# mkocabas/EpipolarPose

Hardware: AMD Instinct MI355X
Metric: images/sec (4-view 256x256, ResNet-50) at 1/2/4/8 MI355X; MPJPE vs ref (higher is better)
Workload: dtype bf16; 1 GPU; configs[1]: ResNet-50 Integral-pose, 4-view 256x256 synthetic, batch=32/GPU, fully-supervised SmoothL1 loss; global_batch=32, joints=17, depth_res=64, optimizer=adam, parallelism=dp1, launch=eager, streams=2, deterministic=True

## Files before the change

### epipolarpose_amd/csrc/common.h

```cpp
#pragma once
#include <hip/hip_runtime.h>
#include <stdint.h>
#include <float.h>
#include "../../include/epipolar_hip.h"

#define EPI_WAVE 64
#define EPI_HD __host__ __device__
#define EPI_LOG2E 1.4426950408889634f

#define EPI_CHECK_LAUNCH()                                   \
    do {                                                     \
        if (hipGetLastError() != hipSuccess) return EPI_ERR_LAUNCH; \
    } while (0)

namespace epi {

typedef float float4v __attribute__((ext_vector_type(4)));
typedef unsigned int uint4v __attribute__((ext_vector_type(4)));

bool deterministic();
float* det_scratch(size_t floats, hipStream_t stream);

__device__ __forceinline__ float fast_exp2(float x) { return __builtin_amdgcn_exp2f(x); }

// ... 35 lines not shown
    __device__ static __forceinline__ void store(unsigned short* p, const float (&v)[8]) {
        unsigned int w[4];
#pragma unroll
        for (int i = 0; i < 4; ++i)
            w[i] = pack_bf16x2(v[2 * i], v[2 * i + 1]);
        uint4v t; t.x = w[0]; t.y = w[1]; t.z = w[2]; t.w = w[3];
        *reinterpret_cast<uint4v*>(p) = t;
    }
    __device__ static __forceinline__ float load1(const unsigned short* p) { return bf16_to_f32(*p); }
    __device__ static __forceinline__ void store1(unsigned short* p, float v) { *p = f32_to_bf16(v); }
};

__device__ __forceinline__ float wave_sum(float v) {
#pragma unroll
    for (int o = 32; o > 0; o >>= 1) v += __shfl_xor(v, o, 64);
    return v;
}
__device__ __forceinline__ float wave_max(float v) {
#pragma unroll
    for (int o = 32; o > 0; o >>= 1) v = fmaxf(v, __shfl_xor(v, o, 64));
    return v;
}

__device__ __forceinline__ float block_sum(float v, float* smem ) {
    const int lane = threadIdx.x & 63, wid = threadIdx.x >> 6, nw = (blockDim.x + 63) >> 6;
    v = wave_sum(v);
    __syncthreads();
    if (lane == 0) smem[wid] = v;
    __syncthreads();
    float t = (lane < nw) ? smem[lane] : 0.f;
    t = wave_sum(t);
    return t;
}

}
```

### epipolarpose_amd/csrc/head_gemm.hip

```cpp
#include "common.h"
#include "bn_affine.h"
#include <algorithm>
#include <cstdlib>
#include <mutex>
#include <type_traits>
#include <unordered_map>
#include <utility>
#include <vector>

namespace epi {

typedef __bf16 bf16x8 __attribute__((ext_vector_type(8)));
typedef float f32x16 __attribute__((ext_vector_type(16)));

constexpr int GBK = 64;

template <int TM_, int WM_, int WN_, int MIN_WAVES_, int NSTAGE_, bool STAGGER_ = false> struct GemmCfg {
    static constexpr int TM = TM_, WM = WM_, WN = WN_, NW = WM_ * WN_, THREADS = 64 * NW, MIN_WAVES = MIN_WAVES_, NSTAGE = NSTAGE_;
    static constexpr bool STAGGER = STAGGER_;
    static constexpr int BM = WM_ * TM_ * 32, BN = WN_ * 64;
    static constexpr int A_BYTES = BM * 128, B_BYTES = BN * 128, STAGE_BYTES = A_BYTES + B_BYTES;
    static constexpr int AP = BM / 8 / NW, BP = BN / 8 / NW;
    static constexpr bool EARLY = NW == 4 && NSTAGE_ == 2;
    static_assert(AP >= 1 && BP >= 1 && BM % (8 * NW) == 0 && BN % (8 * NW) == 0, "whole pieces per wave");
// ... 102 lines not shown
        c.sh[4 * h] = sh.x; c.sh[4 * h + 1] = sh.y; c.sh[4 * h + 2] = sh.z; c.sh[4 * h + 3] = sh.w;
    }
}
__device__ __forceinline__ uint4v bnred_apply(const GemmBnRed& br, uint4v o, uint4v zv, uint4v yv, const BnRedCols& c, float (&s)[8], float (&q)[8]);
__device__ __forceinline__ uint4v bnred_row(const GemmBnRed& br, uint4v o, long long off, const BnRedCols& c, float (&s)[8], float (&q)[8]) {
    const uint4v zv = *reinterpret_cast<const uint4v*>(br.z + off);
    uint4v yv = uint4v{0u, 0u, 0u, 0u};
    if (br.relu && br.y) yv = *reinterpret_cast<const uint4v*>(br.y + off);
    return bnred_apply(br, o, zv, yv, c, s, q);
}
__device__ __forceinline__ uint4v bnred_apply(const GemmBnRed& br, uint4v o, uint4v zv, uint4v yv, const BnRedCols& c, float (&s)[8], float (&q)[8]) {
    unsigned int ow[4] = {o.x, o.y, o.z, o.w};
    const unsigned int zw[4] = {zv.x, zv.y, zv.z, zv.w}, yw[4] = {yv.x, yv.y, yv.z, yv.w};
#pragma unroll
    for (int k = 0; k < 4; ++k) {
#pragma unroll
        for (int h = 0; h < 2; ++h) {
            const int e = 2 * k + h;
            const unsigned int keep = h ? 0xffff0000u : 0x0000ffffu;
            const float g = __uint_as_float(h ? (ow[k] & 0xffff0000u) : (ow[k] << 16));
            const float xv = __uint_as_float(h ? (zw[k] & 0xffff0000u) : (zw[k] << 16));
            bool on = true;
            if (br.relu) on = br.y ? (__uint_as_float(h ? (yw[k] & 0xffff0000u) : (yw[k] << 16)) > 0.f) : (xv * c.sc[e] + c.sh[e] > 0.f);
            const float dz = on ? g : 0.f;
            s[e] += dz;
            q[e] = fmaf(dz, (xv - c.mu[e]) * c.rs[e], q[e]);
            if (!on) ow[k] &= ~keep;
        }
    }
    uint4v r; r.x = ow[0]; r.y = ow[1]; r.z = ow[2]; r.w = ow[3];
    return r;
}

#ifdef EPI_GEMM_TRACE
constexpr int GEMM_TRACE_WGS = 8192, GEMM_TRACE_SLOTS = 16;
__device__ unsigned long long epi_gemm_trace[GEMM_TRACE_WGS * GEMM_TRACE_SLOTS];
#define GEMM_STAMP_V(i, v)                                                                                               \
    do {                                                                                                                 \
        const int wg_ = blockIdx.x + gridDim.x * (blockIdx.y + gridDim.y * blockIdx.z);                                  \
        if (threadIdx.x == 0 && wg_ < GEMM_TRACE_WGS) epi_gemm_trace[wg_ * GEMM_TRACE_SLOTS + (i)] = (v);               \
    } while (0)
#define GEMM_STAMP(i) GEMM_STAMP_V(i, __builtin_amdgcn_s_memtime())
#else
#define GEMM_STAMP_V(i, v) do {} while (0)
#define GEMM_STAMP(i) do {} while (0)
#endif
// ... 114 lines not shown
                for (int k = 0; k < 4; ++k) {
                    const float a = __uint_as_float(w4[k] << 16), b = __uint_as_float(w4[k] & 0xffff0000u);
                    ssum[2 * k] += a; ssq[2 * k] = fmaf(a, a, ssq[2 * k]);
                    ssum[2 * k + 1] += b; ssq[2 * k + 1] = fmaf(b, b, ssq[2 * k + 1]);
                }
            }
            uint4v o; o.x = lo.x; o.y = lo.y; o.z = hi.x; o.w = hi.y;
            if (ADD) o = add_bf16x8(o, AD_EARLY ? ad[it] : addend_at(m_first + 8 * it, off));
            if (RED) o = RED_EARLY ? bnred_apply(p.br, o, zpre[it], ypre[it], rcols, ssum, ssq) : bnred_row(p.br, o, off, rcols, ssum, ssq);
            uint4v* dst = reinterpret_cast<uint4v*>(reinterpret_cast<unsigned short*>(p.C) + off);
            if (nt_stores) __builtin_nontemporal_store(o, dst);
            else *dst = o;
        }
    };
    const bool has_stats = !RED && p.stats != nullptr;
    auto copy_sc = [&](auto sc_c) __attribute__((always_inline)) {
        if (has_stats) { if (has_add) copy_rows(std::true_type{}, std::true_type{}, sc_c); else copy_rows(std::true_type{}, std::false_type{}, sc_c); }
        else if (has_add) copy_rows(std::false_type{}, std::true_type{}, sc_c);
        else copy_rows(std::false_type{}, std::false_type{}, sc_c);
    };
    if (scatter) copy_sc(std::true_type{}); else copy_sc(std::false_type{});
    GEMM_STAMP(6);
    if (has_stats || RED) {
#pragma unroll
        for (int k = 0; k < 8; ++k) {
#pragma unroll
            for (int o = 8; o < 64; o <<= 1) { ssum[k] += __shfl_xor(ssum[k], o, 64); ssq[k] += __shfl_xor(ssq[k], o, 64); }
        }
        float* st = reinterpret_cast<float*>(smem + WM * WN * (TM * 32 * 128));
        if (lane < 8) {
            float* row = st + wm * (2 * GBN) + wn * 64 + c8 * 8;
            *reinterpret_cast<float4v*>(row) = float4v{ssum[0], ssum[1], ssum[2], ssum[3]};
            *reinterpret_cast<float4v*>(row + 4) = float4v{ssum[4], ssum[5], ssum[6], ssum[7]};
            *reinterpret_cast<float4v*>(row + GBN) = float4v{ssq[0], ssq[1], ssq[2], ssq[3]};
            *reinterpret_cast<float4v*>(row + GBN + 4) = float4v{ssq[4], ssq[5], ssq[6], ssq[7]};
        }
        __syncthreads();
        float* dst = RED ? p.br.sums : p.stats + (long long)(tile_m % p.stats_copies) * 2 * p.N;
        for (int t = tid; t < 2 * GBN; t += THREADS) {
            float v = 0.f;
#pragma unroll
            for (int w = 0; w < WM; ++w) v += st[w * (2 * GBN) + t];
            const int which = t / GBN, col = n0 + (t % GBN);
            if (col < p.N) atomicAdd(dst + which * p.N + col, v);
        }
    }
#ifdef EPI_GEMM_TRACE
    asm volatile("s_waitcnt vmcnt(0)" ::: "memory");
    GEMM_STAMP(7);
    GEMM_STAMP_V(8, __builtin_amdgcn_s_memrealtime());
#endif
}

enum { A_PLAIN = 0, A_GATHER = 1, A_PHASED = 2 };


__device__ __forceinline__ bf16x8 bn_in_apply(bf16x8 a, const float4v (&t)[4]) {
    const uint4v u = __builtin_bit_cast(uint4v, a);
    const unsigned int w[4] = {u.x, u.y, u.z, u.w};
// ... 375 lines not shown
                        float* c = reinterpret_cast<float*>(p.C) + orow * p.ldc + n;
                        if (n + 3 < p.N) { float4v t; t.x = v[0]; t.y = v[1]; t.z = v[2]; t.w = v[3]; *reinterpret_cast<float4v*>(c) = t; }
                        else for (int e = 0; e < 4 && n + e < p.N; ++e) c[e] = v[e];
                    } else {
                        unsigned short* c = reinterpret_cast<unsigned short*>(p.C) + orow * p.ldc + n;
                        if (p.addend)
                            for (int e = 0; e < 4 && n + e < p.N; ++e) v[e] = bf16_to_f32(f32_to_bf16(v[e])) + bf16_to_f32(p.addend[orow * p.ldc + n + e]);
                        if (n + 3 < p.N) {
                            uint2 t;
                            t.x = pack_bf16x2(v[0], v[1]);
                            t.y = pack_bf16x2(v[2], v[3]);
                            *reinterpret_cast<uint2*>(c) = t;
                        } else for (int e = 0; e < 4 && n + e < p.N; ++e) c[e] = f32_to_bf16(v[e]);
                    }
                }
            }
        }
    }
}

constexpr int AS_WAVES = 8, AS_LOADERS = 2, AS_RING = 3;
constexpr int AS_THREADS = 64 * (AS_WAVES + AS_LOADERS), AS_BM = 32 * AS_WAVES, AS_BN = 64;

template <int KSTEPS>
__global__ __launch_bounds__(AS_THREADS, 1) void head_gemm_astat_kernel(GemmArgs p) {
    constexpr int K = 16 * KSTEPS, ROW_BYTES = 2 * K, CHUNKS = ROW_BYTES / 16;
    constexpr int BTILE = AS_BN * ROW_BYTES;
    constexpr int ROWS_PER_PIECE = 1024 / ROW_BYTES, PIECES = BTILE / 1024 / AS_LOADERS;
    extern __shared__ __attribute__((aligned(16))) char smem[];
    const int tid = threadIdx.x, lane = tid & 63, wid = tid >> 6;
    const bool loader = wid >= AS_WAVES;
    const int frow = lane & 31, fhalf = lane >> 5;
    const int m0 = xcd_remap(blockIdx.x, gridDim.x) * AS_BM + wid * 32;
    const int n_tiles = (p.N + AS_BN - 1) / AS_BN;
    const char* zero_src = reinterpret_cast<const char*>(epi_zero_chunk);
    float* bias_s = reinterpret_cast<float*>(smem + AS_RING * BTILE + AS_WAVES * 4096);
    float* stats_s = bias_s + n_tiles * AS_BN;
    for (int n = tid; n < n_tiles * AS_BN; n += AS_THREADS) bias_s[n] = (p.bias && n < p.N) ? p.bias[n] : 0.f;
    if (p.stats)
        for (int n = tid; n < 2 * n_tiles * AS_BN; n += AS_THREADS) stats_s[n] = 0.f;

    auto issue_b = [&](int nt) {
        const int lw = wid - AS_WAVES;
        char* dst = smem + (nt % AS_RING) * BTILE + lw * (PIECES * 1024);
#pragma unroll 8
        for (int q = 0; q < PIECES; ++q) {
            const int r = (lw * PIECES + q) * ROWS_PER_PIECE + lane / CHUNKS;
            const int chunk = (lane % CHUNKS) ^ (r % CHUNKS);
            const int n = nt * AS_BN + r;
            const void* src = n < p.N ? reinterpret_cast<const void*>(p.Bt + (long long)n * p.ldb + chunk * 8)
                                      : reinterpret_cast<const void*>(zero_src);
            glds16(src, dst + q * 1024);
        }
    };
    bf16x8 af[KSTEPS];
    if (loader) {
        issue_b(0);
        if (n_tiles > 1) issue_b(1);
    } else {
        const int m = m0 + frow;
        const uint4v* arow = reinterpret_cast<const uint4v*>(p.A + (long long)(m < p.M ? m : 0) * p.lda) + fhalf;
#pragma unroll
        for (int ks = 0; ks < KSTEPS; ++ks) {
            uint4v v = arow[2 * ks];
            if (m >= p.M) v.x = v.y = v.z = v.w = 0u;
            af[ks] = __builtin_bit_cast(bf16x8, v);
        }
    }
    __syncthreads();
    if (loader) {
        for (int nt = 0; nt < n_tiles; ++nt) {
            if (nt + 2 < n_tiles) {
                issue_b(nt + 2);
                asm volatile("s_waitcnt vmcnt(%0)\n\ts_barrier" ::"n"(PIECES) : "memory");
            } else {
                asm volatile("s_waitcnt vmcnt(0)\n\ts_barrier" ::: "memory");
            }
        }
        if (p.stats) __builtin_amdgcn_s_barrier();
        return;
    }
    char* stage = smem + AS_RING * BTILE + wid * 4096;
    const int c8 = lane & 7;
    auto slices = [&](auto add_c, auto stats_c) __attribute__((always_inline)) {
    constexpr bool ADD = decltype(add_c)::value, STATS = decltype(stats_c)::value;
    for (int nt = 0; nt < n_tiles; ++nt) {
        f32x16 acc[2];
#pragma unroll
        for (int j = 0; j < 2; ++j)
#pragma unroll
            for (int r = 0; r < 16; ++r) acc[j][r] = 0.f;
        const unsigned slice_off = (unsigned)(nt % AS_RING) * BTILE;
        auto read_b = [&](int ks, uint4v (&f)[2]) {
#pragma unroll
            for (int tj = 0; tj < 2; ++tj) {
                const int r = tj * 32 + frow;
                const unsigned off = (slice_off + r * ROW_BYTES + (((fhalf ^ r) % CHUNKS) << 4)) ^ (unsigned)(((2 * ks) % CHUNKS) << 4);
                f[tj] = *reinterpret_cast<const uint4v*>(smem + off);
            }
        };
        uint4v ad[4];
        auto load_addend = [&]() {
            if (!ADD) return;
#pragma unroll
            for (int it = 0; it < 4; ++it) {
                const int m = m0 + it * 8 + (lane >> 3), nn = nt * AS_BN + (lane & 7) * 8;
                ad[it] = (m < p.M && nn < p.N) ? *reinterpret_cast<const uint4v*>(p.addend + (long long)m * p.ldc + nn) : uint4v{0u, 0u, 0u, 0u};
            }
        };
        if (KSTEPS <= 8) load_addend();
        uint4v fb[3][2];
        read_b(0, fb[0]);
        if (KSTEPS > 1) read_b(1, fb[1]);
#pragma unroll
        for (int ks = 0; ks < KSTEPS; ++ks) {
            if (ks + 2 < KSTEPS) read_b(ks + 2, fb[(ks + 2) % 3]);
            __builtin_amdgcn_sched_barrier(0);
#pragma unroll
            for (int tj = 0; tj < 2; ++tj)
                acc[tj] = __builtin_amdgcn_mfma_f32_32x32x16_bf16(__builtin_bit_cast(bf16x8, fb[ks % 3][tj]), af[ks], acc[tj], 0, 0, 0);
        }
        asm volatile("s_waitcnt lgkmcnt(0)\n\ts_barrier" ::: "memory");
        const int n0 = nt * AS_BN;
#pragma unroll
        for (int tj = 0; tj < 2; ++tj)
#pragma unroll
            for (int q = 0; q < 4; ++q) {
                const int nl = tj * 32 + 8 * q + 4 * fhalf;
                const float4v bv = *reinterpret_cast<const float4v*>(bias_s + n0 + nl);
                const float v0 = acc[tj][4 * q] + bv.x, v1 = acc[tj][4 * q + 1] + bv.y, v2 = acc[tj][4 * q + 2] + bv.z,
                            v3 = acc[tj][4 * q + 3] + bv.w;
                uint2 t;
                t.x = pack_bf16x2(v0, v1);
                t.y = pack_bf16x2(v2, v3);
                const int unit = tj * 8 + 2 * q + fhalf;
                *reinterpret_cast<uint2*>(stage + frow * 128 + ((unit ^ (frow & 15)) << 3)) = t;
            }
        const int n = n0 + c8 * 8;
        float ssum[8], ssq[8];
#pragma unroll
        for (int k = 0; k < 8; ++k) { ssum[k] = 0.f; ssq[k] = 0.f; }
#pragma unroll
        for (int it = 0; it < 4; ++it) {
            const int row = it * 8 + (lane >> 3), sw = row & 15;
            const uint2 lo = *reinterpret_cast<const uint2*>(stage + row * 128 + (((2 * c8) ^ sw) << 3));
            const uint2 hi = *reinterpret_cast<const uint2*>(stage + row * 128 + (((2 * c8 + 1) ^ sw) << 3));
            const int m = m0 + row;
            if (m < p.M && n < p.N) {
                uint4v o; o.x = lo.x; o.y = lo.y; o.z = hi.x; o.w = hi.y;
                if (ADD) o = add_bf16x8(o, KSTEPS <= 8 ? ad[it] : *reinterpret_cast<const uint4v*>(p.addend + (long long)m * p.ldc + n));
                *reinterpret_cast<uint4v*>(reinterpret_cast<unsigned short*>(p.C) + (long long)m * p.ldc + n) = o;
                if (STATS) {
                    const unsigned int w4[4] = {lo.x, lo.y, hi.x, hi.y};
#pragma unroll
                    for (int k = 0; k < 4; ++k) {
                        const float a = __uint_as_float(w4[k] << 16), b = __uint_as_float(w4[k] & 0xffff0000u);
                        ssum[2 * k] += a; ssq[2 * k] = fmaf(a, a, ssq[2 * k]);
                        ssum[2 * k + 1] += b; ssq[2 * k + 1] = fmaf(b, b, ssq[2 * k + 1]);
                    }
                }
            }
        }
        if (STATS) {
#pragma unroll
            for (int k = 0; k < 8; ++k) {
#pragma unroll
                for (int o = 8; o < 64; o <<= 1) { ssum[k] += __shfl_xor(ssum[k], o, 64); ssq[k] += __shfl_xor(ssq[k], o, 64); }
            }
            if (lane < 8) {
#pragma unroll
                for (int k = 0; k < 8; ++k) {
                    atomicAdd(stats_s + n + k, ssum[k]);
                    atomicAdd(stats_s + n_tiles * AS_BN + n + k, ssq[k]);
                }
            }
        }
    }
    };
    if (p.addend) { if (p.stats) slices(std::true_type{}, std::true_type{}); else slices(std::true_type{}, std::false_type{}); }
    else if (p.stats) slices(std::false_type{}, std::true_type{});
    else slices(std::false_type{}, std::false_type{});
    if (p.stats) {
        asm volatile("s_waitcnt lgkmcnt(0)\n\ts_barrier" ::: "memory");
        float* dst = p.stats + (long long)(blockIdx.x % p.stats_copies) * 2 * p.N;
        for (int n = tid; n < p.N; n += 64 * AS_WAVES) {
            atomicAdd(dst + n, stats_s[n]);
            atomicAdd(dst + p.N + n, stats_s[n_tiles * AS_BN + n]);
        }
    }
}

template <int TM_, int WM_, int WN_> struct PatchCfg {
    static constexpr int TM = TM_, WM = WM_, WN = WN_, NW = WM_ * WN_, THREADS = 64 * NW;
    static constexpr int BM = WM_ * TM_ * 32, BN = WN_ * 64, B_BYTES = BN * 128, BP = BN / 8 / NW;
    static_assert(NW == 8 && BP >= 1, "8 waves");
};
typedef PatchCfg<2, 4, 2> PatchWide;
typedef PatchCfg<1, 8, 1> PatchNarrow;
typedef PatchCfg<1, 4, 2> PatchHalf;
constexpr int PATCH_TAPS = 9, PATCH_APW = 8;

#ifdef EPI_PATCH_TRACE
__device__ unsigned long long epi_patch_trace[64 * 96];
#define PATCH_STAMP(i)                                                                                                   \
    do {                                                                                                                 \
        const int wg_ = blockIdx.x + gridDim.x * blockIdx.y;                                                             \
        if (lane == 0 && wid == 0 && wg_ % 16 == 0 && wg_ / 16 < 64 && (i) < 96) epi_patch_trace[(wg_ / 16) * 96 + (i)] = __builtin_amdgcn_s_memtime(); \
// ... 261 lines not shown
static int g_pipe_force_fwd();
static int gemm_pipe_mode() {
    const int v = 0;
    const int f = g_pipe_force_fwd();
    return f >= 0 ? f : v;
}

static int g_store_policy = -1;
static int gemm_store_policy() {
    if (g_store_policy < 0) g_store_policy = 0;
    return g_store_policy;
}
extern "C" int epi_gemm_store_policy(int v) {
    const int before = gemm_store_policy();
    if (v >= 0) g_store_policy = v;
    return before;
}
static int g_tile_force = 0, g_pipe_force = -1;
extern "C" int epi_gemm_tune(int tile, int pipe) {
    if (tile >= 0) g_tile_force = tile;
    if (pipe >= -1) g_pipe_force = pipe;
    return g_tile_force;
}

static int g_tile_force_fwd() { return g_tile_force; }
static int g_pipe_force_fwd() { return g_pipe_force; }

static GemmPlan gemm_plan_cfg(int cfg, int M, int N, int K, int nphase, bool pipe = false) {
    GemmPlan pl;
    pl.cfg = cfg;
    pl.pipe = pipe ? 1 : 0;
    const int bm = cfg == CFG_SMALL ? 128 : (cfg == CFG_HALF || cfg == CFG_QUARTER ? 64 : 256);
    const int bn = cfg == CFG_BIG ? 256 : (cfg == CFG_TALL || cfg == CFG_QUARTER ? 64 : 128);
    pl.tiles = (long long)((M + bm - 1) / bm) * ((N + bn - 1) / bn);
    const long long wgs = pl.tiles * nphase;
    const bool one_per_cu = cfg == CFG_BIG || pipe;
    const long long enough_env = 120;
    const long long enough = enough_env, target = one_per_cu ? 256 : 512;
    int nsplit = 1;
    if (wgs < enough) {
        nsplit = (int)(target / wgs);
        const int max_split = K / 512 > 0 ? K / 512 : 1;
        if (nsplit > max_split) nsplit = max_split;
        if (nsplit > 16) nsplit = 16;
        if (nsplit < 1) nsplit = 1;
    }
// ... 179 lines not shown
    a.coalesce = (!out_f32 && a.N % 8 == 0 && a.ldc % 8 == 0) ? 1 : 0;
    const bool half_addend = a.addend && a.addend_step == 2;
    if (half_addend && (!a.coalesce || a.ga.enabled || a.sc.enabled || a.ph.enabled || nphase != 1 || a.add_h <= 0 || a.add_w <= 0 || ((a.add_h | a.add_w) & 1) ||
                        (long long)a.M % ((long long)a.add_h * a.add_w)))
        return EPI_ERR_UNSUPPORTED;
    const bool fuse_stats = true;
    float* const want_stats = (fuse_stats && !deterministic()) ? a.stats : nullptr;
    a.stats = nullptr;
    if (!a.A || !a.Bt || !a.C || a.M <= 0 || a.N <= 0 || a.K <= 0) return EPI_ERR_INVALID_ARGUMENT;
    if (a.K % 8 || a.ldb % 8 || a.ldc % 4 || (!a.ga.enabled && a.lda % 8)) return EPI_ERR_UNSUPPORTED;
    if ((reinterpret_cast<uintptr_t>(a.A) | reinterpret_cast<uintptr_t>(a.Bt) | reinterpret_cast<uintptr_t>(a.C)) & 15u) return EPI_ERR_UNSUPPORTED;
    if (a.ga.enabled && (a.ga.Cs % GBK)) return EPI_ERR_UNSUPPORTED;
    if (a.bn_in_on) {
        if (out_f32 || a.ga.enabled || a.sc.enabled || a.ph.enabled || nphase != 1 || a.K % GBK || a.K > 2048 || want_red.z || a.bias || a.addend || !a.coalesce ||
            !a.bn_in.gamma || !a.bn_in.beta || !a.bn_in.scale || !a.bn_in.shift)
            return EPI_ERR_UNSUPPORTED;
        const GemmPlan pl = gemm_plan_cfg(CFG_SMALL, a.M, a.N, a.K, 1);
        if (pl.tiles > 0x7fffffffLL) return EPI_ERR_UNSUPPORTED;
        if (pl.nsplit > 1) {
            if (!workspace || (size_t)pl.nsplit * a.M * a.N * sizeof(float) > workspace_bytes) return EPI_ERR_WORKSPACE;
            a.slabs = (float*)workspace;
        }
        a.k_per_split = pl.kps;
        if (want_stats && pl.nsplit == 1) { a.stats = want_stats; if (stats_done) *stats_done = 1; }
        const int rc = launch_gemm_mode<false, CfgSmall, A_PLAIN, false, true>(a, pl, 1, st);
        if (rc != EPI_OK) return rc;
        if (pl.nsplit > 1) {
            if (want_stats && a.N % 4 == 0) {
                a.stats = want_stats;
                if (stats_done) *stats_done = 1;
                const unsigned blocks = (unsigned)(((a.M + FS_ROWS - 1) / FS_ROWS) * ((a.N + 255) / 256));
                hipLaunchKernelGGL(splitk_finish_stats_kernel, dim3(blocks), dim3(256), 0, st, a.slabs, pl.nsplit, a);
            } else {
                const long long n = (long long)a.M * (a.N >> 2);
                hipLaunchKernelGGL(splitk_finish_kernel<false>, dim3((unsigned)((n + 255) / 256)), dim3(256), 0, st, a.slabs, pl.nsplit, 1, a);
            }
            EPI_CHECK_LAUNCH();
        }
        return EPI_OK;
    }
    const bool stats_off_astat = true;
    if (!want_red.z && !(want_stats && stats_off_astat && !a.bias) && !half_addend &&
        !out_f32 && !a.ga.enabled && !a.sc.enabled && nphase == 1 && (a.K == 64 || a.K == 128 || a.K == 256) && a.N % 8 == 0 &&
        a.ldc % 8 == 0 && a.N >= 4 * AS_BN && a.N <= 8192 && a.M >= 64 * AS_BM && gemm_tile_override() == 0) {
        const unsigned grid = (unsigned)((a.M + AS_BM - 1) / AS_BM);
        const bool astat_stats = false;
        if (want_stats && !a.bias && astat_stats) { a.stats = want_stats; if (stats_done) *stats_done = 1; }
#define EPI_ASTAT(KS)                                                                                                      \
        do {                                                                                                               \
            const size_t lds = AS_RING * (size_t)AS_BN * 32 * KS + AS_WAVES * 4096 + (size_t)((a.N + AS_BN - 1) / AS_BN) * AS_BN * 4 * 3;                                          \
            static const hipError_t attr = hipFuncSetAttribute(reinterpret_cast<const void*>(&head_gemm_astat_kernel<KS>),  \
                                                               hipFuncAttributeMaxDynamicSharedMemorySize, (int)lds);      \
            if (attr != hipSuccess) return EPI_ERR_LAUNCH;                                                                 \
            hipLaunchKernelGGL((head_gemm_astat_kernel<KS>), dim3(grid), dim3(AS_THREADS), lds, st, a);                     \
        } while (0)
        if (a.K == 256) EPI_ASTAT(16);
        else if (a.K == 128) EPI_ASTAT(8);
        else EPI_ASTAT(4);
#undef EPI_ASTAT
        EPI_CHECK_LAUNCH();
        return EPI_OK;
    }
    if (patch_eligible(a, out_f32, nphase)) {
        const PatchPlan pp = patch_plan(a.M, a.N, a.ga.Cs, a.ga.Wg, workspace ? workspace_bytes : 0);
        if (pp.ok) {
            a.patch_px = pp.patch_px;
            a.chunks_per_split = pp.cps;
            if (pp.nsplit > 1) a.slabs = (float*)workspace;
            else if (want_stats) { a.stats = want_stats; if (stats_done) *stats_done = 1; }
            else if (want_red.z) { a.br = want_red; *red_done = 1; }
            int rc;
            if (pp.cfg == PATCH_NARROW && pp.single) rc = pp.nb == 3 ? launch_patch<PatchNarrow, 3, true>(a, pp, st) : launch_patch<PatchNarrow, 2, true>(a, pp, st);
            else if (pp.cfg == PATCH_NARROW) rc = pp.nb == 3 ? launch_patch<PatchNarrow, 3>(a, pp, st) : launch_patch<PatchNarrow, 2>(a, pp, st);
            else if (pp.cfg == PATCH_HALF) rc = pp.nb == 3 ? launch_patch<PatchHalf, 3>(a, pp, st) : launch_patch<PatchHalf, 2>(a, pp, st);
            else rc = pp.nb == 3 ? launch_patch<PatchWide, 3>(a, pp, st) : launch_patch<PatchWide, 2>(a, pp, st);
            if (rc != EPI_OK) return rc;
            if (pp.nsplit > 1) {
                if (want_stats && !a.addend) {
                    a.stats = want_stats;
                    if (stats_done) *stats_done = 1;
                    const unsigned blocks = (unsigned)(((a.M + FS_ROWS - 1) / FS_ROWS) * ((a.N + 255) / 256));
                    hipLaunchKernelGGL(splitk_finish_stats_kernel, dim3(blocks), dim3(256), 0, st, a.slabs, pp.nsplit, a);
                } else {
                    const long long n = (long long)a.M * (a.N >> 2);
                    hipLaunchKernelGGL(splitk_finish_kernel<false>, dim3((unsigned)((n + 255) / 256)), dim3(256), 0, st, a.slabs, pp.nsplit, 1, a);
                }
                EPI_CHECK_LAUNCH();
            }
            return EPI_OK;
        }
    }
    GemmPlan pl = gemm_plan(a.M, a.N, a.K, a.ldc, nphase, out_f32);
    if (want_red.z && pl.pipe && pl.cfg != CFG_SMALL) pl = gemm_plan(a.M, a.N, a.K, a.ldc, nphase, out_f32, false);
    if (pl.tiles > 0x7fffffffLL) return EPI_ERR_UNSUPPORTED;
    if (half_addend && pl.nsplit > 1) return EPI_ERR_UNSUPPORTED;
    if (pl.nsplit > 1) {
        if (!workspace || (size_t)pl.nsplit * nphase * a.M * a.N * sizeof(float) > workspace_bytes) return EPI_ERR_WORKSPACE;
        a.slabs = (float*)workspace;
    }
    a.k_per_split = pl.kps;
    if (want_stats && pl.nsplit == 1 && a.coalesce && !a.bias) { a.stats = want_stats; if (stats_done) *stats_done = 1; }
    if (want_red.z && pl.nsplit == 1 && a.coalesce && (!pl.pipe || pl.cfg == CFG_SMALL) && (pl.cfg == CFG_BIG || pl.cfg == CFG_SMALL || pl.cfg == CFG_TALL)) {
        a.br = want_red;
        *red_done = 1;
    }
    int rc;
    if (a.br.z) rc = pl.cfg == CFG_BIG ? launch_gemm_cfg<false, CfgBig, true>(a, pl, nphase, st)
                   : (pl.cfg == CFG_TALL ? launch_gemm_cfg<false, CfgTall, true>(a, pl, nphase, st)
                      : (pl.pipe ? launch_gemm_cfg<false, CfgSmallP, true>(a, pl, nphase, st) : launch_gemm_cfg<false, CfgSmall, true>(a, pl, nphase, st)));
    else if (pl.cfg == CFG_BIG) rc = g_tile_force == 5 ? launch_gemm_cfg<false, CfgBigLock>(a, pl, nphase, st) : launch_gemm_cfg<false, CfgBig>(a, pl, nphase, st);
    else if (out_f32) rc = launch_gemm_cfg<true, CfgSmall>(a, pl, nphase, st);
    else if (pl.cfg == CFG_HALF) rc = launch_gemm_cfg<false, CfgHalf>(a, pl, nphase, st);
    else if (pl.cfg == CFG_QUARTER) rc = launch_gemm_cfg<false, CfgQuarter>(a, pl, nphase, st);
    else if (pl.cfg == CFG_TALL) rc = pl.pipe ? launch_gemm_cfg<false, CfgTallP>(a, pl, nphase, st) : launch_gemm_cfg<false, CfgTall>(a, pl, nphase, st);
    else rc = pl.pipe ? launch_gemm_cfg<false, CfgSmallP>(a, pl, nphase, st) : launch_gemm_cfg<false, CfgSmall>(a, pl, nphase, st);
    if (rc != EPI_OK) return rc;
    if (pl.nsplit > 1) {
        const long long n = (long long)nphase * a.M * (a.N >> 2);
        const dim3 fg((unsigned)((n + 255) / 256));
        if (!out_f32 && want_stats && nphase == 1 && !a.bias && !a.addend && !a.sc.enabled && !a.ph.enabled && a.N % 4 == 0) {
            a.stats = want_stats;
            if (stats_done) *stats_done = 1;
            const unsigned blocks = (unsigned)(((a.M + FS_ROWS - 1) / FS_ROWS) * ((a.N + 255) / 256));
// ... 1258 lines not shown
```

### epipolarpose_amd/hip.py

```python
import ctypes
import os

import torch

_LIB_DIR = os.environ.get("EPI_LIB_DIR") or os.path.join(os.path.dirname(os.path.abspath(__file__)), "_lib")
_LIB_PATH = os.path.join(_LIB_DIR, "libepipolar_hip.so")
_lib = None

EPI_F32, EPI_BF16, EPI_F64 = 0, 1, 2
EPI_NCHW, EPI_NHWC = 0, 1
LOSS_KINDS = {"l1": 0, "l2": 1, "smoothl1": 2}
TRI_METHODS = {"iterative": 0, "ls": 1, "dlt": 2, "poly": 3}

_vp, _i, _d, _sz = ctypes.c_void_p, ctypes.c_int, ctypes.c_double, ctypes.c_size_t


class EpiViewMeta(ctypes.Structure):
    _fields_ = [(k, _vp) for k in ("center_x", "center_y", "width", "height", "scale", "rot", "R", "T", "f", "c", "P")]


_SIGNATURES = {
    "epi_version": (ctypes.c_char_p, []),
    "epi_status_string": (ctypes.c_char_p, [_i]),
    "epi_softargmax3d_workspace_bytes": (_sz, [_i] * 5),
# ... 29 lines not shown
    "epi_conv2d_pack_fill_row": (_i, [_vp, _vp, _vp, _i, _i, _i, _i, _i, _i, ctypes.c_longlong, ctypes.POINTER(ctypes.c_longlong)]),
    "epi_conv2d_pack_weight_bwd_multi": (_i, [_vp, _i, ctypes.c_longlong, _vp]),
    "epi_conv2d_bwd_data": (_i, [_vp, _vp, _vp, _i, _i, _i, _i, _i, _i, _i, _i, _i, _vp, _vp, _sz, _vp]),
    "epi_conv2d_bwd_data_bnred": (_i, [_vp, _vp, _vp, _i, _i, _i, _i, _i, _i, _i, _i, _i, _vp, _i, _vp, _vp, _vp, _sz, _vp]),
    "epi_conv2d_bwd_data_half_addend_ok": (_i, [_i, _i, _i, _i, _i]),
    "epi_deconv4x4s2_bwd_data_bnred": (_i, [_vp, _vp, _vp, _i, _i, _i, _i, _i, _vp, _vp, _vp, _sz, _vp]),
    "epi_gemm_bf16_bnred": (_i, [_vp, _i, _vp, _i, _vp, _i, _i, _i, _i, _vp, _vp, _vp, _sz, _vp]),
    "epi_bn_finalize": (_i, [_vp, ctypes.c_longlong, _i, ctypes.c_float, ctypes.c_float, _i, _vp]),
    "epi_maxpool3x3s2_bn_relu_fwd": (_i, [_vp, _vp, _vp, _vp, _i, _i, _i, _i, _vp]),
    "epi_bn_act_fwd_dual": (_i, [_vp, _vp, ctypes.c_longlong, _i, _vp, _vp, ctypes.c_float, ctypes.c_float, _i, _vp, _vp]),
    "epi_bn_act_bwd_reduced": (_i, [_vp, _vp, ctypes.c_longlong, _i, _vp, _vp, _vp, _vp, _vp, _vp, _vp, _vp, _vp]),
    "epi_conv2d_bwd_weight": (_i, [_vp, _vp, _vp, _i, _i, _i, _i, _i, _i, _i, _i, _i, _i, _vp, ctypes.c_size_t, _vp]),
    "epi_conv2d_bwd_weight_deferred": (_i, [_vp, _vp, _vp, _i, _i, _i, _i, _i, _i, _i, _i, _i, _i, _vp, ctypes.c_size_t, _vp, _vp]),
    "epi_slab_reduce_chunks": (ctypes.c_longlong, [ctypes.c_longlong]),
    "epi_slab_reduce_multi": (_i, [_vp, _i, ctypes.c_longlong, _vp]),
    "epi_wgrad_group_max": (_i, []),
    "epi_wgrad_group_plan": (_i, [_vp, _i, ctypes.POINTER(ctypes.c_size_t), ctypes.POINTER(ctypes.c_int)]),
    "epi_wgrad_group": (_i, [_vp, _i, _vp, _sz, _vp, _vp]),
    "epi_wgrad_item": (_i, [_vp, _vp, _sz, _vp, _vp]),
    "epi_bn_sum_copies": (_i, [_i]),
    "epi_conv3x3_patch_mode": (_i, [_i]),
    "epi_gemm_tune": (_i, [_i, _i]),
    "epi_gemm_store_policy": (_i, [_i]),
    "epi_set_deterministic": (_i, [_i]),
    "epi_bn_act_fwd": (_i, [_vp, _vp, ctypes.c_longlong, _i, _vp, _vp, ctypes.c_float, ctypes.c_float, _i, _i, _vp, _vp, _vp, _vp,
                            _vp, _vp, _vp, _vp, _vp, _vp]),
    "epi_bn_act_bwd": (_i, [_vp, _vp, _vp, ctypes.c_longlong, _i, _vp, _vp, _vp, _vp, _i, _vp, _vp, _vp, _vp, _vp, _vp]),
    "epi_gemm_tn_workspace_bytes": (_sz, [_i, _i, _i, _i]),
    "epi_gemm_tn_plan": (_i, [_i, _i, _i, _i, ctypes.POINTER(ctypes.c_longlong)]),
    "epi_gemm_tn_bf16": (_i, [_vp, _i, _vp, _i, _vp, _i, _i, _i, _vp, _sz, _vp]),
    "epi_deconv4x4s2_bwd_weight": (_i, [_vp, _vp, _vp, _i, _i, _i, _i, _i, _i, _vp, _sz, _vp]),
    "epi_deconv4x4s2_pack_phase_cl": (_i, [_vp, _i, _i, _vp, _vp]),
    "epi_deconv4x4s2_pack_fill_row": (_i, [_vp, _vp, _vp, _i, _i, ctypes.c_longlong, ctypes.POINTER(ctypes.c_longlong)]),
    "epi_column_sums_bf16": (_i, [_vp, ctypes.c_longlong, _i, _vp, _vp]),
    "epi_stem7x7s2_s2d_bytes": (_sz, [_i, _i, _i]),
    "epi_stem7x7s2_workspace_bytes": (_sz, [_i, _i, _i, _i]),
    "epi_stem7x7s2_s2d": (_i, [_vp, _i, _i, _i, _i, _i, _vp, _vp]),
    "epi_stem7x7s2_pack_weight": (_i, [_vp, _i, _i, _vp, _vp]),
    "epi_stem7x7s2_unpack_weight_grad": (_i, [_vp, _i, _i, _vp, _i, _vp]),
    "epi_stem7x7s2_fwd": (_i, [_vp, _vp, _vp, _i, _i, _i, _i, _vp, _vp, _vp, _sz, _vp]),
    "epi_stem7x7s2_bwd_weight": (_i, [_vp, _vp, _vp, _i, _i, _i, _i, _vp, _sz, _vp]),
    "epi_split_bf16": (_i, [_vp, ctypes.c_longlong, _i, _vp, _i, _i, _vp, _vp]),
    "epi_conv2d_fwd_f32": (_i, [_vp, _vp, _vp, _i, _i, _i, _i, _i, _i, _i, _i, _i, _vp, _sz, _vp]),
    "epi_conv2d_bwd_data_f32": (_i, [_vp, _vp, _vp, _i, _i, _i, _i, _i, _i, _i, _i, _i, _vp, _sz, _vp]),
    "epi_deconv4x4s2_fwd_f32": (_i, [_vp, _vp, _vp, _i, _i, _i, _i, _i, _vp, _sz, _vp]),
    "epi_deconv4x4s2_bwd_data_f32": (_i, [_vp, _vp, _vp, _i, _i, _i, _i, _i, _vp, _sz, _vp]),
# ... 897 lines not shown
```

### include/epipolar_hip.h

```cpp
#ifndef EPIPOLAR_HIP_H
#define EPIPOLAR_HIP_H

#include <stddef.h>
#include <stdint.h>

#ifdef __cplusplus
extern "C" {
#endif

typedef void* epi_stream_t;

enum epi_status {
    EPI_OK = 0,
    EPI_ERR_INVALID_ARGUMENT = 1,
    EPI_ERR_UNSUPPORTED = 2,
    EPI_ERR_WORKSPACE = 3,
    EPI_ERR_LAUNCH = 4
};

enum epi_dtype { EPI_F32 = 0, EPI_BF16 = 1, EPI_F64 = 2 };
enum epi_layout {
    EPI_NCHW = 0,
    EPI_NHWC = 1
};
// ... 119 lines not shown
typedef struct EpiBnReduce {
    const void* z;
    const void* y;
    const float* bn;
    float* sums;
    int relu;
} EpiBnReduce;
int epi_bn_act_bwd_reduced(const void* dz, const void* x, long long R, int C, const float* gamma, const float* mean, const float* rstd,
                           const float* scale_shift, const float* dbeta_dgamma, void* dx, float* fwd_sums_clear, float* param_grads,
                           epi_stream_t stream);
int epi_conv2d_bwd_data_bnred(const void* dy, const void* w_bwd, void* dx, int B, int H, int W, int Cin, int Cout, int KH, int KW,
                              int stride, int pad, const void* addend, int addend_step, const EpiBnReduce* red, int* red_done, void* workspace,
                              size_t workspace_bytes, epi_stream_t stream);
int epi_conv2d_bwd_data_half_addend_ok(int B, int H, int W, int Cin, int Cout);
int epi_deconv4x4s2_bwd_data_bnred(const void* dy, const void* w_bwd, void* dx, int B, int H, int W, int Cin, int Cout,
                                   const EpiBnReduce* red, int* red_done, void* workspace, size_t workspace_bytes, epi_stream_t stream);
int epi_gemm_bf16_bnred(const void* A, int lda, const void* Bt, int ldb, void* C, int ldc, int M, int N, int K, const EpiBnReduce* red,
                        int* red_done, void* workspace, size_t workspace_bytes, epi_stream_t stream);

size_t epi_conv2d_workspace_bytes(int B, int H, int W, int Cin, int Cout, int KH, int KW, int stride, int pad);
int epi_conv3x3_patch_mode(int mode);
int epi_gemm_tune(int tile, int pipe);
int epi_gemm_store_policy(int policy);
int epi_conv2d_fwd(const void* x, const void* w, void* y, int B, int H, int W, int Cin, int Cout, int KH, int KW,
                   int stride, int pad, float* bn_sums, int* bn_sums_done, void* workspace, size_t workspace_bytes,
                   epi_stream_t stream);
int epi_conv1x1_fwd_bn_in(const void* z, const EpiBnLayer* in_bn, int in_training, float eps, float momentum, const void* w, void* y, int B, int H, int W,
                          int Cin, int Cout, float* bn_sums, int* bn_sums_done, void* workspace, size_t workspace_bytes, epi_stream_t stream);
int epi_conv2d_pack_weight_bwd(const void* w, int Cout, int Cin, int KH, int KW, int stride, int pad, void* w_bwd,
                               epi_stream_t stream);
size_t epi_conv2d_pack_row_bytes(void);
int epi_conv2d_pack_fill_row(void* row_host, const void* w, void* w_bwd, int Cout, int Cin, int KH, int KW, int stride, int pad,
                             long long tile_begin, long long* ntiles);
int epi_conv2d_pack_weight_bwd_multi(const void* rows, int nrows, long long total_tiles, epi_stream_t stream);
int epi_conv2d_bwd_data(const void* dy, const void* w_bwd, void* dx, int B, int H, int W, int Cin, int Cout, int KH, int KW,
                        int stride, int pad, const void* addend, void* workspace, size_t workspace_bytes, epi_stream_t stream);

int epi_conv2d_bwd_weight(const void* x, const void* dy, void* dw, int dw_dtype, int B, int H, int W, int Cin, int Cout,
                          int KH, int KW, int stride, int pad, void* workspace, size_t workspace_bytes, epi_stream_t stream);
typedef struct EpiSlabReduce {
    const float* slabs;
    void* out;
    long long n;
    long long chunk_begin;
    int nsplit, out_bf16;
} EpiSlabReduce;
// ... 87 lines not shown
```

Baseline: 2897 images/s.

## Fuse BN-backward column reduction into astat GEMM for K=64 and use permlane butterfly

Extends the A-stationary head GEMM with a RED template path so K=64 GEMMs that need a fused batch-norm backward reduction can use it instead of falling back to the generic tiled kernel. It preloads z/y operands before the MFMA loop, shortens the B prefetch depth to free registers, and applies the relu mask plus sum/sum-of-squares accumulation in the epilogue. The per-column wave reduction is replaced by a permlane32/permlane16/DPP butterfly that spreads the final values across lanes, cutting shuffle count and per-lane atomic pressure. The cost is higher register and LDS pressure in the fused variant and a reduced prefetch distance, which may slow the MFMA loop. A fusion toggle and a last-kernel query are added for control.

```diff
diff --git a/epipolarpose_amd/csrc/common.h b/epipolarpose_amd/csrc/common.h
--- a/epipolarpose_amd/csrc/common.h
+++ b/epipolarpose_amd/csrc/common.h
@@ -81,6 +81,28 @@
     return v;
 }
 
+__device__ __forceinline__ int colsum_k0(int lane) { return ((lane >> 3) & 1) * 2 + ((lane >> 4) & 1) * 4; }
+__device__ __forceinline__ void colsum_butterfly(const float (&s)[8], const float (&q)[8], int lane, float (&out)[2]) {
+    typedef unsigned int uint2v __attribute__((ext_vector_type(2)));
+    float w[8], x[4];
+#pragma unroll
+    for (int k = 0; k < 8; ++k) {
+        const uint2v r = __builtin_amdgcn_permlane32_swap(__float_as_uint(s[k]), __float_as_uint(q[k]), false, false);
+        w[k] = __uint_as_float(r[0]) + __uint_as_float(r[1]);
+    }
+#pragma unroll
+    for (int k = 0; k < 4; ++k) {
+        const uint2v r = __builtin_amdgcn_permlane16_swap(__float_as_uint(w[k]), __float_as_uint(w[k + 4]), false, false);
+        x[k] = __uint_as_float(r[0]) + __uint_as_float(r[1]);
+    }
+    const bool up = (lane & 8) != 0;
+#pragma unroll
+    for (int k = 0; k < 2; ++k) {
+        const float keep = up ? x[k + 2] : x[k], give = up ? x[k] : x[k + 2];
+        out[k] = keep + __uint_as_float((unsigned int)__builtin_amdgcn_update_dpp(0, (int)__float_as_uint(give), 0x128, 0xf, 0xf, false));
+    }
+}
+
 __device__ __forceinline__ float block_sum(float v, float* smem ) {
     const int lane = threadIdx.x & 63, wid = threadIdx.x >> 6, nw = (blockDim.x + 63) >> 6;
     v = wave_sum(v);
diff --git a/epipolarpose_amd/csrc/head_gemm.hip b/epipolarpose_amd/csrc/head_gemm.hip
--- a/epipolarpose_amd/csrc/head_gemm.hip
+++ b/epipolarpose_amd/csrc/head_gemm.hip
@@ -148,6 +148,30 @@
             const float xv = __uint_as_float(h ? (zw[k] & 0xffff0000u) : (zw[k] << 16));
             bool on = true;
             if (br.relu) on = br.y ? (__uint_as_float(h ? (yw[k] & 0xffff0000u) : (yw[k] << 16)) > 0.f) : (xv * c.sc[e] + c.sh[e] > 0.f);
+            const float dz = on ? g : 0.f;
+            s[e] += dz;
+            q[e] = fmaf(dz, (xv - c.mu[e]) * c.rs[e], q[e]);
+            if (!on) ow[k] &= ~keep;
+        }
+    }
+    uint4v r; r.x = ow[0]; r.y = ow[1]; r.z = ow[2]; r.w = ow[3];
+    return r;
+}
+template <int MASK>
+__device__ __forceinline__ uint4v bnred_apply_fixed(uint4v o, uint4v zv, uint4v yv, const BnRedCols& c, float (&s)[8], float (&q)[8]) {
+    unsigned int ow[4] = {o.x, o.y, o.z, o.w};
+    const unsigned int zw[4] = {zv.x, zv.y, zv.z, zv.w}, yw[4] = {yv.x, yv.y, yv.z, yv.w};
+#pragma unroll
+    for (int k = 0; k < 4; ++k) {
+#pragma unroll
+        for (int h = 0; h < 2; ++h) {
+            const int e = 2 * k + h;
+            const unsigned int keep = h ? 0xffff0000u : 0x0000ffffu;
+            const float g = __uint_as_float(h ? (ow[k] & 0xffff0000u) : (ow[k] << 16));
+            const float xv = __uint_as_float(h ? (zw[k] & 0xffff0000u) : (zw[k] << 16));
+            bool on = true;
+            if (MASK == 1) on = __uint_as_float(h ? (yw[k] & 0xffff0000u) : (yw[k] << 16)) > 0.f;
+            if (MASK == 2) on = xv * c.sc[e] + c.sh[e] > 0.f;
             const float dz = on ? g : 0.f;
             s[e] += dz;
             q[e] = fmaf(dz, (xv - c.mu[e]) * c.rs[e], q[e]);
@@ -308,19 +332,10 @@
     if (scatter) copy_sc(std::true_type{}); else copy_sc(std::false_type{});
     GEMM_STAMP(6);
     if (has_stats || RED) {
-#pragma unroll
-        for (int k = 0; k < 8; ++k) {
-#pragma unroll
-            for (int o = 8; o < 64; o <<= 1) { ssum[k] += __shfl_xor(ssum[k], o, 64); ssq[k] += __shfl_xor(ssq[k], o, 64); }
-        }
+        float fin[2];
+        colsum_butterfly(ssum, ssq, lane, fin);
         float* st = reinterpret_cast<float*>(smem + WM * WN * (TM * 32 * 128));
-        if (lane < 8) {
-            float* row = st + wm * (2 * GBN) + wn * 64 + c8 * 8;
-            *reinterpret_cast<float4v*>(row) = float4v{ssum[0], ssum[1], ssum[2], ssum[3]};
-            *reinterpret_cast<float4v*>(row + 4) = float4v{ssum[4], ssum[5], ssum[6], ssum[7]};
-            *reinterpret_cast<float4v*>(row + GBN) = float4v{ssq[0], ssq[1], ssq[2], ssq[3]};
-            *reinterpret_cast<float4v*>(row + GBN + 4) = float4v{ssq[4], ssq[5], ssq[6], ssq[7]};
-        }
+        *reinterpret_cast<float2*>(st + wm * (2 * GBN) + (lane >> 5) * GBN + wn * 64 + c8 * 8 + colsum_k0(lane)) = float2{fin[0], fin[1]};
         __syncthreads();
         float* dst = RED ? p.br.sums : p.stats + (long long)(tile_m % p.stats_copies) * 2 * p.N;
         for (int t = tid; t < 2 * GBN; t += THREADS) {
@@ -742,8 +757,9 @@
 constexpr int AS_WAVES = 8, AS_LOADERS = 2, AS_RING = 3;
 constexpr int AS_THREADS = 64 * (AS_WAVES + AS_LOADERS), AS_BM = 32 * AS_WAVES, AS_BN = 64;
 
-template <int KSTEPS>
+template <int KSTEPS, bool RED = false>
 __global__ __launch_bounds__(AS_THREADS, 1) void head_gemm_astat_kernel(GemmArgs p) {
+    static_assert(!RED || KSTEPS <= 4, "the fused reduction needs the registers the K = 128 / 256 fragments hold");
     constexpr int K = 16 * KSTEPS, ROW_BYTES = 2 * K, CHUNKS = ROW_BYTES / 16;
     constexpr int BTILE = AS_BN * ROW_BYTES;
     constexpr int ROWS_PER_PIECE = 1024 / ROW_BYTES, PIECES = BTILE / 1024 / AS_LOADERS;
@@ -756,9 +772,17 @@
     const char* zero_src = reinterpret_cast<const char*>(epi_zero_chunk);
     float* bias_s = reinterpret_cast<float*>(smem + AS_RING * BTILE + AS_WAVES * 4096);
     float* stats_s = bias_s + n_tiles * AS_BN;
+    float* bn_s = stats_s + 2 * n_tiles * AS_BN;
+    const GemmBnRed br = p.br;
+    const bool col_sums = RED || p.stats != nullptr;
     for (int n = tid; n < n_tiles * AS_BN; n += AS_THREADS) bias_s[n] = (p.bias && n < p.N) ? p.bias[n] : 0.f;
-    if (p.stats)
+    if (col_sums)
         for (int n = tid; n < 2 * n_tiles * AS_BN; n += AS_THREADS) stats_s[n] = 0.f;
+    if (RED)
+        for (int n = tid; n < 4 * n_tiles * AS_BN; n += AS_THREADS) {
+            const int which = n / (n_tiles * AS_BN), col = n - which * (n_tiles * AS_BN);
+            bn_s[n] = col < p.N ? br.bn[which * p.N + col] : 0.f;
+        }
 
     auto issue_b = [&](int nt) {
         const int lw = wid - AS_WAVES;
@@ -797,13 +821,14 @@
                 asm volatile("s_waitcnt vmcnt(0)\n\ts_barrier" ::: "memory");
             }
         }
-        if (p.stats) __builtin_amdgcn_s_barrier();
+        if (col_sums) __builtin_amdgcn_s_barrier();
         return;
     }
     char* stage = smem + AS_RING * BTILE + wid * 4096;
     const int c8 = lane & 7;
-    auto slices = [&](auto add_c, auto stats_c) __attribute__((always_inline)) {
+    auto slices = [&](auto add_c, auto stats_c, auto mask_c) __attribute__((always_inline)) {
     constexpr bool ADD = decltype(add_c)::value, STATS = decltype(stats_c)::value;
+    constexpr int MASK = decltype(mask_c)::value;
     for (int nt = 0; nt < n_tiles; ++nt) {
         f32x16 acc[2];
 #pragma unroll
@@ -828,18 +853,31 @@
                 ad[it] = (m < p.M && nn < p.N) ? *reinterpret_cast<const uint4v*>(p.addend + (long long)m * p.ldc + nn) : uint4v{0u, 0u, 0u, 0u};
             }
         };
-        if (KSTEPS <= 8) load_addend();
-        uint4v fb[3][2];
+        if (KSTEPS <= 8 && !RED) load_addend();
+        uint4v zpre[RED ? 4 : 1], ypre[RED && MASK == 1 ? 4 : 1];
+        if (RED) {
+#pragma unroll
+            for (int it = 0; it < 4; ++it) {
+                const int m = m0 + it * 8 + (lane >> 3), nn = nt * AS_BN + (lane & 7) * 8;
+                const bool ok = m < p.M && nn < p.N;
+                const long long off = (long long)m * p.ldc + nn;
+                zpre[it] = ok ? *reinterpret_cast<const uint4v*>(br.z + off) : uint4v{0u, 0u, 0u, 0u};
+                if (MASK == 1) ypre[it] = ok ? *reinterpret_cast<const uint4v*>(br.y + off) : uint4v{0u, 0u, 0u, 0u};
+            }
+        }
+        constexpr int AHEAD = RED ? 1 : 2;
+        uint4v fb[AHEAD + 1][2];
         read_b(0, fb[0]);
-        if (KSTEPS > 1) read_b(1, fb[1]);
+        if (KSTEPS > 1 && AHEAD > 1) read_b(1, fb[1]);
 #pragma unroll
         for (int ks = 0; ks < KSTEPS; ++ks) {
-            if (ks + 2 < KSTEPS) read_b(ks + 2, fb[(ks + 2) % 3]);
+            if (ks + AHEAD < KSTEPS) read_b(ks + AHEAD, fb[(ks + AHEAD) % (AHEAD + 1)]);
             __builtin_amdgcn_sched_barrier(0);
 #pragma unroll
             for (int tj = 0; tj < 2; ++tj)
-                acc[tj] = __builtin_amdgcn_mfma_f32_32x32x16_bf16(__builtin_bit_cast(bf16x8, fb[ks % 3][tj]), af[ks], acc[tj], 0, 0, 0);
-        }
+                acc[tj] = __builtin_amdgcn_mfma_f32_32x32x16_bf16(__builtin_bit_cast(bf16x8, fb[ks % (AHEAD + 1)][tj]), af[ks], acc[tj], 0, 0, 0);
+        }
+        if (RED) load_addend();
         asm volatile("s_waitcnt lgkmcnt(0)\n\ts_barrier" ::: "memory");
         const int n0 = nt * AS_BN;
 #pragma unroll
@@ -860,6 +898,21 @@
         float ssum[8], ssq[8];
 #pragma unroll
         for (int k = 0; k < 8; ++k) { ssum[k] = 0.f; ssq[k] = 0.f; }
+        BnRedCols rcols;
+        if (RED) {
+            const int nc = n_tiles * AS_BN;
+#pragma unroll
+            for (int h = 0; h < 2; ++h) {
+                const float4v zero = float4v{0.f, 0.f, 0.f, 0.f};
+                const float4v mu = *reinterpret_cast<const float4v*>(bn_s + n + 4 * h), rs = *reinterpret_cast<const float4v*>(bn_s + nc + n + 4 * h);
+                const float4v sc = MASK != 2 ? zero : *reinterpret_cast<const float4v*>(bn_s + 2 * nc + n + 4 * h);
+                const float4v sh = MASK != 2 ? zero : *reinterpret_cast<const float4v*>(bn_s + 3 * nc + n + 4 * h);
+                rcols.mu[4 * h] = mu.x; rcols.mu[4 * h + 1] = mu.y; rcols.mu[4 * h + 2] = mu.z; rcols.mu[4 * h + 3] = mu.w;
+                rcols.rs[4 * h] = rs.x; rcols.rs[4 * h + 1] = rs.y; rcols.rs[4 * h + 2] = rs.z; rcols.rs[4 * h + 3] = rs.w;
+                rcols.sc[4 * h] = sc.x; rcols.sc[4 * h + 1] = sc.y; rcols.sc[4 * h + 2] = sc.z; rcols.sc[4 * h + 3] = sc.w;
+                rcols.sh[4 * h] = sh.x; rcols.sh[4 * h + 1] = sh.y; rcols.sh[4 * h + 2] = sh.z; rcols.sh[4 * h + 3] = sh.w;
+            }
+        }
 #pragma unroll
         for (int it = 0; it < 4; ++it) {
             const int row = it * 8 + (lane >> 3), sw = row & 15;
@@ -869,6 +922,7 @@
             if (m < p.M && n < p.N) {
                 uint4v o; o.x = lo.x; o.y = lo.y; o.z = hi.x; o.w = hi.y;
                 if (ADD) o = add_bf16x8(o, KSTEPS <= 8 ? ad[it] : *reinterpret_cast<const uint4v*>(p.addend + (long long)m * p.ldc + n));
+                if (RED) o = bnred_apply_fixed<MASK>(o, zpre[it], ypre[MASK == 1 ? it : 0], rcols, ssum, ssq);
                 *reinterpret_cast<uint4v*>(reinterpret_cast<unsigned short*>(p.C) + (long long)m * p.ldc + n) = o;
                 if (STATS) {
                     const unsigned int w4[4] = {lo.x, lo.y, hi.x, hi.y};
@@ -881,28 +935,29 @@
                 }
             }
         }
-        if (STATS) {
-#pragma unroll
-            for (int k = 0; k < 8; ++k) {
-#pragma unroll
-                for (int o = 8; o < 64; o <<= 1) { ssum[k] += __shfl_xor(ssum[k], o, 64); ssq[k] += __shfl_xor(ssq[k], o, 64); }
-            }
-            if (lane < 8) {
-#pragma unroll
-                for (int k = 0; k < 8; ++k) {
-                    atomicAdd(stats_s + n + k, ssum[k]);
-                    atomicAdd(stats_s + n_tiles * AS_BN + n + k, ssq[k]);
-                }
-            }
+        if (STATS || RED) {
+            float fin[2];
+            colsum_butterfly(ssum, ssq, lane, fin);
+            float* col = stats_s + (lane >> 5) * (n_tiles * AS_BN) + n + colsum_k0(lane);
+            atomicAdd(col, fin[0]);
+            atomicAdd(col + 1, fin[1]);
         }
     }
     };
-    if (p.addend) { if (p.stats) slices(std::true_type{}, std::true_type{}); else slices(std::true_type{}, std::false_type{}); }
-    else if (p.stats) slices(std::false_type{}, std::true_type{});
-    else slices(std::false_type{}, std::false_type{});
-    if (p.stats) {
+    typedef std::integral_constant<int, 0> mask0;
+    if (RED) {
+        auto red_slices = [&](auto mask_c) __attribute__((always_inline)) {
+            if (p.addend) slices(std::true_type{}, std::false_type{}, mask_c); else slices(std::false_type{}, std::false_type{}, mask_c);
+        };
+        if (!br.relu) red_slices(mask0{});
+        else if (br.y) red_slices(std::integral_constant<int, 1>{});
+        else red_slices(std::integral_constant<int, 2>{});
+    } else if (p.addend) { if (p.stats) slices(std::true_type{}, std::true_type{}, mask0{}); else slices(std::true_type{}, std::false_type{}, mask0{}); }
+    else if (p.stats) slices(std::false_type{}, std::true_type{}, mask0{});
+    else slices(std::false_type{}, std::false_type{}, mask0{});
+    if (col_sums) {
         asm volatile("s_waitcnt lgkmcnt(0)\n\ts_barrier" ::: "memory");
-        float* dst = p.stats + (long long)(blockIdx.x % p.stats_copies) * 2 * p.N;
+        float* dst = RED ? br.sums : p.stats + (long long)(blockIdx.x % p.stats_copies) * 2 * p.N;
         for (int n = tid; n < p.N; n += 64 * AS_WAVES) {
             atomicAdd(dst + n, stats_s[n]);
             atomicAdd(dst + p.N + n, stats_s[n_tiles * AS_BN + n]);
@@ -1210,6 +1265,16 @@
     if (pipe >= -1) g_pipe_force = pipe;
     return g_tile_force;
 }
+
+enum { ASTAT_RED_K64 = 1 };
+static int g_astat_fusions = ASTAT_RED_K64;
+extern "C" int epi_gemm_astat_fusions(int mask) {
+    const int before = g_astat_fusions;
+    if (mask >= 0) g_astat_fusions = mask & 1;
+    return before;
+}
+static int g_last_kernel = EPI_GEMM_KERNEL_NONE;
+extern "C" int epi_gemm_last_kernel(void) { return g_last_kernel; }
 
 static int g_tile_force_fwd() { return g_tile_force; }
 static int g_pipe_force_fwd() { return g_pipe_force; }
@@ -1435,6 +1500,7 @@
             a.slabs = (float*)workspace;
         }
         a.k_per_split = pl.kps;
+        g_last_kernel = EPI_GEMM_KERNEL_GENERIC;
         if (want_stats && pl.nsplit == 1) { a.stats = want_stats; if (stats_done) *stats_done = 1; }
         const int rc = launch_gemm_mode<false, CfgSmall, A_PLAIN, false, true>(a, pl, 1, st);
         if (rc != EPI_OK) return rc;
@@ -1452,24 +1518,29 @@
         }
         return EPI_OK;
     }
-    const bool stats_off_astat = true;
-    if (!want_red.z && !(want_stats && stats_off_astat && !a.bias) && !half_addend &&
+    const bool stats_off_astat = want_stats && !a.bias;
+    const bool astat_red = want_red.z && a.K == 64 && (g_astat_fusions & ASTAT_RED_K64);
+    if ((!want_red.z || astat_red) && !stats_off_astat && !half_addend &&
         !out_f32 && !a.ga.enabled && !a.sc.enabled && nphase == 1 && (a.K == 64 || a.K == 128 || a.K == 256) && a.N % 8 == 0 &&
         a.ldc % 8 == 0 && a.N >= 4 * AS_BN && a.N <= 8192 && a.M >= 64 * AS_BM && gemm_tile_override() == 0) {
         const unsigned grid = (unsigned)((a.M + AS_BM - 1) / AS_BM);
-        const bool astat_stats = false;
-        if (want_stats && !a.bias && astat_stats) { a.stats = want_stats; if (stats_done) *stats_done = 1; }
-#define EPI_ASTAT(KS)                                                                                                      \
+        g_last_kernel = EPI_GEMM_KERNEL_ASTAT;
+#define EPI_ASTAT(KS, RED)                                                                                                 \
         do {                                                                                                               \
-            const size_t lds = AS_RING * (size_t)AS_BN * 32 * KS + AS_WAVES * 4096 + (size_t)((a.N + AS_BN - 1) / AS_BN) * AS_BN * 4 * 3;                                          \
-            static const hipError_t attr = hipFuncSetAttribute(reinterpret_cast<const void*>(&head_gemm_astat_kernel<KS>),  \
-                                                               hipFuncAttributeMaxDynamicSharedMemorySize, (int)lds);      \
+            const size_t lds = AS_RING * (size_t)AS_BN * 32 * KS + AS_WAVES * 4096 + (size_t)((a.N + AS_BN - 1) / AS_BN) * AS_BN * 4 * (RED ? 7 : 3); \
+            if (lds > 160 * 1024) return EPI_ERR_UNSUPPORTED;                                                              \
+            static const hipError_t attr = hipFuncSetAttribute(reinterpret_cast<const void*>(&head_gemm_astat_kernel<KS, RED>), \
+                                                               hipFuncAttributeMaxDynamicSharedMemorySize, 160 * 1024);    \
             if (attr != hipSuccess) return EPI_ERR_LAUNCH;                                                                 \
-            hipLaunchKernelGGL((head_gemm_astat_kernel<KS>), dim3(grid), dim3(AS_THREADS), lds, st, a);                     \
+            hipLaunchKernelGGL((head_gemm_astat_kernel<KS, RED>), dim3(grid), dim3(AS_THREADS), lds, st, a);                \
         } while (0)
-        if (a.K == 256) EPI_ASTAT(16);
-        else if (a.K == 128) EPI_ASTAT(8);
-        else EPI_ASTAT(4);
+        if (astat_red) {
+            a.br = want_red;
+            *red_done = 1;
+            EPI_ASTAT(4, true);
+        } else if (a.K == 256) EPI_ASTAT(16, false);
+        else if (a.K == 128) EPI_ASTAT(8, false);
+        else EPI_ASTAT(4, false);
 #undef EPI_ASTAT
         EPI_CHECK_LAUNCH();
         return EPI_OK;
@@ -1477,6 +1548,7 @@
     if (patch_eligible(a, out_f32, nphase)) {
         const PatchPlan pp = patch_plan(a.M, a.N, a.ga.Cs, a.ga.Wg, workspace ? workspace_bytes : 0);
         if (pp.ok) {
+            g_last_kernel = EPI_GEMM_KERNEL_PATCH;
             a.patch_px = pp.patch_px;
             a.chunks_per_split = pp.cps;
             if (pp.nsplit > 1) a.slabs = (float*)workspace;
@@ -1512,6 +1584,7 @@
         a.slabs = (float*)workspace;
     }
     a.k_per_split = pl.kps;
+    g_last_kernel = EPI_GEMM_KERNEL_GENERIC;
     if (want_stats && pl.nsplit == 1 && a.coalesce && !a.bias) { a.stats = want_stats; if (stats_done) *stats_done = 1; }
     if (want_red.z && pl.nsplit == 1 && a.coalesce && (!pl.pipe || pl.cfg == CFG_SMALL) && (pl.cfg == CFG_BIG || pl.cfg == CFG_SMALL || pl.cfg == CFG_TALL)) {
         a.br = want_red;
diff --git a/epipolarpose_amd/hip.py b/epipolarpose_amd/hip.py
--- a/epipolarpose_amd/hip.py
+++ b/epipolarpose_amd/hip.py
@@ -75,6 +75,8 @@
     "epi_conv3x3_patch_mode": (_i, [_i]),
     "epi_gemm_tune": (_i, [_i, _i]),
     "epi_gemm_store_policy": (_i, [_i]),
+    "epi_gemm_astat_fusions": (_i, [_i]),
+    "epi_gemm_last_kernel": (_i, []),
     "epi_set_deterministic": (_i, [_i]),
     "epi_bn_act_fwd": (_i, [_vp, _vp, ctypes.c_longlong, _i, _vp, _vp, ctypes.c_float, ctypes.c_float, _i, _i, _vp, _vp, _vp, _vp,
                             _vp, _vp, _vp, _vp, _vp, _vp]),
diff --git a/include/epipolar_hip.h b/include/epipolar_hip.h
--- a/include/epipolar_hip.h
+++ b/include/epipolar_hip.h
@@ -165,6 +165,9 @@
 int epi_conv3x3_patch_mode(int mode);
 int epi_gemm_tune(int tile, int pipe);
 int epi_gemm_store_policy(int policy);
+enum { EPI_GEMM_KERNEL_NONE = 0, EPI_GEMM_KERNEL_GENERIC = 1, EPI_GEMM_KERNEL_ASTAT = 2, EPI_GEMM_KERNEL_PATCH = 3 };
+int epi_gemm_astat_fusions(int mask);
+int epi_gemm_last_kernel(void);
 int epi_conv2d_fwd(const void* x, const void* w, void* y, int B, int H, int W, int Cin, int Cout, int KH, int KW,
                    int stride, int pad, float* bn_sums, int* bn_sums_done, void* workspace, size_t workspace_bytes,
                    epi_stream_t stream);
```

Measured after the change: 2887 images/s. No clear change (-0.3%).
